# PREDICT-EPFL/polympc

Measured on AMD Instinct MI355X. Metric: box-ADMM QP subproblem solves/s (fused SQP hot path), higher is better.
Workload: dtype f64

## Files before the change

polympc_amd/csrc/pmpc_qp_reg.hpp:

```cpp
#pragma once
#include <hip/hip_runtime.h>
#include "pmpc_qp.hpp"

#ifndef PMPC_REG_RESIDUAL_BATCH
#define PMPC_REG_RESIDUAL_BATCH 14
#endif

namespace pmpc {

__device__ __forceinline__ double bcast_lane(double v, int lane) {
    const int lo = __builtin_amdgcn_readlane(__double2loint(v), lane);
    const int hi = __builtin_amdgcn_readlane(__double2hiint(v), lane);
    return __hiloint2double(hi, lo);
}
__device__ __forceinline__ void lds_order() { asm volatile("" ::: "memory"); }
__device__ __forceinline__ void sched_fence() { __builtin_amdgcn_sched_barrier(0); }

#ifndef PMPC_PIVOT_SETUP_FORM
#define PMPC_PIVOT_SETUP_FORM 0
#endif
__device__ __forceinline__ void pivot_lane_setup(double& a0, double& a1, double& a2, double& a3, double& a4, double& a5, double& a6, double& l,
                                                 double lk, int k) {
    asm("s_lshl_b64 exec, 1, %9\n\tv_mov_b64 %0, 0\n\tv_mov_b64 %1, 0\n\tv_mov_b64 %2, 0\n\tv_mov_b64 %3, 0\n\tv_mov_b64 %4, 0\n\tv_mov_b64 %5, 0\n\t"
        "v_mov_b64 %6, 0\n\tv_mov_b64 %7, %8\n\ts_mov_b64 exec, -1"
        : "+v"(a0), "+v"(a1), "+v"(a2), "+v"(a3), "+v"(a4), "+v"(a5), "+v"(a6), "+v"(l) : "v"(lk), "i"(k) : "scc");
}
__device__ __forceinline__ void pivot_lane_setup(double& a0, double& a1, double& a2, double& l, double lk, int k) {
#if PMPC_PIVOT_SETUP_FORM == 1
    asm volatile("s_lshl_b64 exec, 1, %5\n\tv_mov_b64 %0, 0\n\tv_mov_b64 %1, 0\n\tv_mov_b64 %2, 0\n\tv_mov_b64 %3, %4\n\ts_mov_b64 exec, -1"
        : "+v"(a0), "+v"(a1), "+v"(a2), "+v"(l) : "v"(lk), "i"(k) : "scc");
#elif PMPC_PIVOT_SETUP_FORM == 2
    unsigned long long saved, win;
    asm volatile("s_mov_b64 %4, exec\n\ts_lshl_b64 %5, 1, %7\n\ts_and_b64 exec, %4, %5\n\tv_mov_b64 %0, 0\n\tv_mov_b64 %1, 0\n\tv_mov_b64 %2, 0\n\tv_mov_b64 %3, %6\n\ts_mov_b64 exec, %4"
        : "+v"(a0), "+v"(a1), "+v"(a2), "+v"(l), "=&s"(saved), "=&s"(win) : "v"(lk), "i"(k) : "scc");
#elif PMPC_PIVOT_SETUP_FORM == 3
    const bool me = lane_id() == k;
    a0 = me ? 0.0 : a0; a1 = me ? 0.0 : a1; a2 = me ? 0.0 : a2; l = me ? lk : l;
#else
    asm("s_lshl_b64 exec, 1, %5\n\tv_mov_b64 %0, 0\n\tv_mov_b64 %1, 0\n\tv_mov_b64 %2, 0\n\tv_mov_b64 %3, %4\n\ts_mov_b64 exec, -1"
        : "+v"(a0), "+v"(a1), "+v"(a2), "+v"(l) : "v"(lk), "i"(k) : "scc");
#endif
}
__device__ __forceinline__ double recip_uniform(double d) {
    double y = __builtin_amdgcn_rcp(d);
    y = fma(fma(-d, y, 1.0), y, y);
    y = fma(fma(-d, y, 1.0), y, y);
    y = fma(fma(-d, y, 1.0), y, y);
    return __builtin_amdgcn_div_fixup(y, d, 1.0);
}

template <int J>
__device__ __forceinline__ double fmac_rowbcast(double acc, double x, double w) {
    asm("v_fmac_f64_dpp %0, %1, %2 row_newbcast:%3 row_mask:0xf bank_mask:0xf" : "+v"(acc) : "v"(x), "v"(w), "i"(J));
    return acc;
}
__device__ __forceinline__ void swap32(double& a, double& b) {
    const auto lo = __builtin_amdgcn_permlane32_swap(__double2loint(a), __double2loint(b), false, false);
    const auto hi = __builtin_amdgcn_permlane32_swap(__double2hiint(a), __double2hiint(b), false, false);
    a = __hiloint2double(hi[0], lo[0]); b = __hiloint2double(hi[1], lo[1]);
}
__device__ __forceinline__ void swap16(double& a, double& b) {
    const auto lo = __builtin_amdgcn_permlane16_swap(__double2loint(a), __double2loint(b), false, false);
    const auto hi = __builtin_amdgcn_permlane16_swap(__double2hiint(a), __double2hiint(b), false, false);
    a = __hiloint2double(hi[0], lo[0]); b = __hiloint2double(hi[1], lo[1]);
}

template <int N>
struct RegKkt {
    double a[((N + 15) / 16) * 16];
    using d4 = double __attribute__((ext_vector_type(4)));
    static constexpr int BK = 4;
    static constexpr int SG = 8;
    static constexpr int NB = (N + BK - 1) / BK;
    static constexpr int NT = (N + 15) / 16;
    static constexpr int NP = NT * 16;
    static constexpr int SK = 80;
    static constexpr int SX = SG + 1;
    static constexpr int XSZ = (64 * SX + 64 > BK * SK) ? 64 * SX + 64 : BK * SK;
    static constexpr int SY = 78;
    static constexpr int TRI = (BK * SK + XSZ > 16 * SY) ? BK * SK + XSZ : 16 * SY;
    static_assert(N <= 64 && SK % 32 == 16 && SK >= 64, "panel stride");
    static_assert(16 * SY <= TRI && BK % 4 == 0 && 16 % BK == 0 && BK <= SG, "conversion buffer fits the staging; block size divides a tile");

    struct NoPre { template <class TT> __device__ __forceinline__ void operator()(TT&, double*, double*, int, int, int) const {} };
    template <int NLIVE>
    __device__ __forceinline__ static double diag_abs_max(const d4 (&T)[NT][NT], int lr, int lc) {
        double dm = 0.0;
#pragma unroll
        for (int R = 0; R < (NLIVE + 15) / 16; ++R)
#pragma unroll
            for (int r = 0; r < 4; ++r) dm = fmax(dm, (lc == lr + 4 * r && 16 * R + lc < NLIVE) ? fabs(T[R][R][r]) : 0.0);
        return wave_max(dm);
    }
    template <int MM, class ALoad, class RhoOf>
    __device__ __forceinline__ static void rank_update(d4 (&T)[NT][NT], int ln, int lr, int lc, double* PA, double* PB, ALoad aload, RhoOf rho_of) {
        constexpr int NGR = (MM + 3) / 4, GB = 4;
        int z = 0;
        asm volatile("" : "+v"(z));
#pragma unroll
        for (int g0 = 0; g0 < NGR; g0 += GB) {
            double av_[GB * 4];
#pragma unroll
            for (int u = 0; u < GB * 4; ++u) { const int j = 4 * g0 + u; av_[u] = (j < MM) ? aload(j < MM ? j : 0, z) : 0.0; }
            sched_fence();
#pragma unroll
            for (int gg = 0; gg < GB; ++gg) {
                if (g0 + gg < NGR) {
#pragma unroll
                    for (int t = 0; t < 4; ++t) {
                        const int j = 4 * (g0 + gg) + t;
                        const double rj = (j < MM) ? rho_of(j < MM ? j : 0) : 0.0;
                        PB[t * SK + ln] = av_[gg * 4 + t];
                        PA[t * SK + ln] = rj * av_[gg * 4 + t];
                    }
                    lds_order();
                    double av[NT], bv[NT];
#pragma unroll
                    for (int R = 0; R < NT; ++R) { av[R] = PA[lr * SK + 16 * R + lc]; bv[R] = PB[lr * SK + 16 * R + lc]; }
                    bool nz[NT]; double probe = 0.0;
#pragma unroll
                    for (int R = 0; R < NT; ++R) { nz[R] = __builtin_amdgcn_ballot_w64(bv[R] != 0.0) != 0; probe += (av[R] - av[R]) + (bv[R] - bv[R]); }
                    const bool all = __builtin_amdgcn_ballot_w64(probe != 0.0) != 0;
#pragma unroll
                    for (int R = 0; R < NT; ++R)
#pragma unroll
                        for (int C = 0; C <= R; ++C)
                            if (all || (nz[R] && nz[C])) T[R][C] = __builtin_amdgcn_mfma_f64_16x16x4f64(av[R], bv[C], T[R][C], 0, 0, 0);
                    sched_fence();
                    lds_order();
                }
            }
        }
    }
    template <int NPIV = N, bool EST = false, class KCol, class Pre = NoPre>
    __device__ __forceinline__ bool invert(int ln_in, double* st, double diag, KCol kcol, long long* tm = nullptr, double rho_self = 0.0, Pre pre = Pre(), const double gate = PMPC_COND_GATE) {
        constexpr bool CF = NPIV < N;
        constexpr int NBP = (NPIV + BK - 1) / BK;
        long long tq0 = tm ? clock64() : 0;
        int ln = ln_in;
        asm volatile("" : "+v"(ln));
        double* PA = st;
        double* PB = st + BK * SK;
        double* X = PB;
        const int lr = ln >> 4, lc = ln & 15;
        d4 T[NT][NT];
        X[64 * SX + ln] = diag;
        sched_fence();
        int z = 0;
        asm volatile("" : "+v"(z));
#pragma unroll
        for (int j = 0; j < NP; ++j) a[j] = (j < N) ? kcol(j < N ? j : 0, z) : 0.0;
        sched_fence();
        const bool isPl = ln < NPIV;
        if constexpr (CF) {
#pragma unroll
            for (int j = 0; j < NPIV; ++j) { const double sc = -(rho_self * a[j]); a[j] = isPl ? a[j] : sc; }
        }
#pragma unroll
        for (int g = 0; g < NP / SG; ++g) {
#pragma unroll
            for (int t = 0; t < SG; ++t) {
                double v = a[g * SG + t];
                if constexpr (CF) {
                    if (g * SG + t >= NPIV && g * SG + t < N && 16 * ((g * SG + t) / 16) < NPIV) { const double sc = -(bcast_lane(rho_self, (g * SG + t < N) ? g * SG + t : 0) * v); v = isPl ? sc : v; }
                }
                X[ln * SX + t] = v;
            }
            lds_order();
            if ((lc >> 3) == (g % 2)) {
#pragma unroll
                for (int R = g / 2; R < NT; ++R)
#pragma unroll
                    for (int r = 0; r < 4; ++r) T[R][g / 2][r] = X[(16 * R + lr + 4 * r) * SX + (lc & 7)];
            }
            lds_order();
            sched_fence();
        }
#pragma unroll
        for (int R = 0; R < NT; ++R) {
            const double dR = X[64 * SX + 16 * R + lc];
#pragma unroll
            for (int r = 0; r < 4; ++r) T[R][R][r] = (lc == lr + 4 * r) ? dR : T[R][R][r];
        }
        lds_order();
        if constexpr (CF) {
            constexpr int MC = N - NPIV, KS = (MC + 3) / 4, NTP = (NPIV + 15) / 16;
#pragma unroll
            for (int s2 = 0; s2 < KS; ++s2) {
#pragma unroll
                for (int t = 0; t < 4; ++t) {
                    const int j = 4 * s2 + t;
                    const double raw = (j < MC) ? a[(NPIV + j < NP) ? NPIV + j : 0] : 0.0;
                    const double rj = (j < MC) ? bcast_lane(rho_self, (NPIV + j < N) ? NPIV + j : 0) : 0.0;
                    const double pa = rj * raw;
                    PA[t * SK + ln] = (isPl && j < MC) ? pa : 0.0;
                    PB[t * SK + ln] = (isPl && j < MC) ? raw : 0.0;
                }
                lds_order();
                double av[NTP], bv[NTP];
#pragma unroll
                for (int R = 0; R < NTP; ++R) { av[R] = PA[lr * SK + 16 * R + lc]; bv[R] = PB[lr * SK + 16 * R + lc]; }
#pragma unroll
                for (int R = 0; R < NTP; ++R)
#pragma unroll
                    for (int C = 0; C <= R; ++C) T[R][C] = __builtin_amdgcn_mfma_f64_16x16x4f64(av[R], bv[C], T[R][C], 0, 0, 0);
                sched_fence();
                lds_order();
            }
        }
        pre(T, PA, PB, ln, lr, lc);
        if constexpr (EST) { X[64 * SX + ln] = diag_abs_max<NPIV>(T, lr, lc); lds_order(); }
        if (tm) { long long t = clock64(); tm[0] += t - tq0; tq0 = t; }
#pragma unroll
        for (int b = 0; b < NBP; ++b) {
            const int kb = b * BK;
            const int w = (NPIV - kb < BK) ? NPIV - kb : BK;
            const int Cb = kb / 16, hb = (kb % 16) / BK;
            constexpr int RPB = BK / 4;
            if ((lc / BK) == hb) {
#pragma unroll
                for (int R = Cb; R < NT; ++R)
#pragma unroll
                    for (int r = 0; r < 4; ++r) X[(16 * R + lr + 4 * r) * SX + (lc % BK)] = T[R][Cb][r];
            }
#pragma unroll
            for (int C = 0; C < Cb; ++C)
#pragma unroll
                for (int rr = 0; rr < RPB; ++rr) X[(16 * C + lc) * SX + lr + 4 * rr] = T[Cb][C][RPB * hb + rr];
            lds_order();
            double p[BK];
#pragma unroll
            for (int t = 0; t < BK; ++t) p[t] = X[ln * SX + t];
            lds_order();
            const bool inb = (ln / BK) == b && (!CF || ln < NPIV);
            if (tm) { long long t = clock64(); tm[1] += t - tq0; tq0 = t; }
#pragma unroll
            for (int t = 0; t < BK; ++t) PB[t * SK + ln] = (inb || kb + t >= NPIV) ? 0.0 : p[t];
#pragma unroll
            for (int t = 0; t < BK; ++t) {
                const int k = kb + t;
                if (k < NPIV) {
                    const double dk = bcast_lane(p[t], k);
                    const double r = recip_uniform(dk);
                    double rk[BK];
#pragma unroll
                    for (int u = 0; u < BK; ++u) rk[u] = (u != t && u < w) ? bcast_lane(p[u], k) : 0.0;
                    double l = p[t] * r;
                    if (w == BK) {
                        if constexpr (BK == 8) pivot_lane_setup(p[(t + 1) & 7], p[(t + 2) & 7], p[(t + 3) & 7], p[(t + 4) & 7], p[(t + 5) & 7], p[(t + 6) & 7], p[(t + 7) & 7], l, -r, k);
                        else pivot_lane_setup(p[(t + 1) & 3], p[(t + 2) & 3], p[(t + 3) & 3], l, -r, k);
                    } else {
#pragma unroll
                        for (int u = 0; u < BK; ++u) if (u != t && u < w) p[u] = (ln == k) ? 0.0 : p[u];
                        l = (ln == k) ? -r : l;
                    }
#pragma unroll
                    for (int u = 0; u < BK; ++u)
                        if (u != t && u < w) p[u] = fma(-l, rk[u], p[u]);
                    p[t] = l;
                    sched_fence();
                }
            }
            if (tm) { long long t = clock64(); tm[2] += t - tq0; tq0 = t; }
#pragma unroll
            for (int t = 0; t < BK; ++t) PA[t * SK + ln] = (inb || kb + t >= NPIV) ? 0.0 : -p[t];
            lds_order();
#pragma unroll
            for (int s2 = 0; s2 < BK / 4; ++s2) {
                double av[NT], bv[NT];
#pragma unroll
                for (int R = 0; R < NT; ++R) {
                    av[R] = PA[(4 * s2 + lr) * SK + 16 * R + lc];
                    bv[R] = PB[(4 * s2 + lr) * SK + 16 * R + lc];
                }
#pragma unroll
                for (int R = 0; R < NT; ++R)
#pragma unroll
                    for (int C = 0; C <= R; ++C) T[R][C] = __builtin_amdgcn_mfma_f64_16x16x4f64(av[R], bv[C], T[R][C], 0, 0, 0);
                sched_fence();
            }
            lds_order();
            if (tm) { long long t = clock64(); tm[3] += t - tq0; tq0 = t; }
#pragma unroll
            for (int t = 0; t < BK; ++t) X[ln * SX + t] = p[t];
            lds_order();
            if ((lc / BK) == hb && (lc % BK) < w) {
#pragma unroll
                for (int R = Cb; R < NT; ++R)
#pragma unroll
                    for (int r = 0; r < 4; ++r) T[R][Cb][r] = X[(16 * R + lr + 4 * r) * SX + (lc % BK)];
            }
#pragma unroll
            for (int C = 0; C <= Cb; ++C)
#pragma unroll
                for (int rr = 0; rr < RPB; ++rr) {
                    const double xv_ = X[(16 * C + lc) * SX + lr + 4 * rr];
                    T[Cb][C][RPB * hb + rr] = (w == BK || lr + 4 * rr < w) ? xv_ : T[Cb][C][RPB * hb + rr];
                }
            lds_order();
            sched_fence();
        }
        if (tm) { long long t = clock64(); tm[1] += t - tq0; tq0 = t; }
        if constexpr (EST) {
            const double smax = X[64 * SX + ln];
            const double wmax = diag_abs_max<NPIV>(T, lr, lc);
            if (__builtin_amdgcn_readfirstlane((int)(smax * wmax > gate))) return true;
        }
        double* Y = st;
#pragma unroll
        for (int q = 0; q < NT; ++q) {
#pragma unroll
            for (int C = 0; C < NT; ++C) {
                if (C <= q) {
#pragma unroll
                    for (int r = 0; r < 4; ++r) Y[(lr + 4 * r) * SY + 16 * C + lc] = T[q][C][r];
                } else {
#pragma unroll
                    for (int r = 0; r < 4; ++r) Y[lc * SY + 16 * C + lr + 4 * r] = T[C][q][r];
                }
            }
            lds_order();
            const int yo = lc * SY + 16 * (lr < NT ? lr : 0);
#pragma unroll
            for (int j = 0; j < 16; ++j) {
                const double y = Y[yo + j];
                a[16 * q + j] = (16 * (NT - 1) + j < N && NT == 4) ? y : ((16 * lr + j < N) ? y : 0.0);
            }
            lds_order();
            sched_fence();
        }
        if (tm) { long long t = clock64(); tm[4] += t - tq0; tq0 = t; }
        return false;
    }

    __device__ __forceinline__ double apply(double c) const {
        double acc[4] = {0.0, 0.0, 0.0, 0.0};
        asm volatile("s_nop 1" : "+v"(c));
        unroll_j<0>(acc, c);
        asm volatile("s_nop 1" : "+v"(acc[0]), "+v"(acc[1]), "+v"(acc[2]), "+v"(acc[3]));
        swap32(acc[0], acc[2]);
        swap32(acc[1], acc[3]);
        double s0 = acc[0] + acc[2], s1 = acc[1] + acc[3];
        swap16(s0, s1);
        return -(s0 + s1);
    }
    template <int J>
    __device__ __forceinline__ void unroll_j(double (&acc)[4], double c) const {
        if constexpr (J < 16) {
#pragma unroll
            for (int q = 0; q < NT; ++q) acc[q] = fmac_rowbcast<J>(acc[q], c, a[16 * q + J]);
            unroll_j<J + 1>(acc, c);
        }
    }
};

template <int NN, int MM, bool STACKED = false, bool SYMLOWER = false, bool GATE = false>
__device__ __forceinline__ void boxadmm_solve_reg(const double* __restrict__ H, const double* h, const double* __restrict__ A,
                                                  const double* Alb, const double* Aub, const double* xlb, const double* xub,
                                                  const double* x0, const double* y0, const pmpc_qp_settings& s, pmpc_qp_info& info,
                                                  double* out_x, double* out_y, double* tr, long long* dbg = nullptr, long long* tm = nullptr) {
    constexpr int N = NN + MM;
    static_assert(N <= WAVE, "register-resident path needs n+m <= 64");
    const long long tp0 = dbg ? clock64() : 0;
    const int ln = lane_id();
    const bool isP = ln < NN;
    const bool isC = (ln >= NN) && (ln < N);
    const int r = isC ? ln - NN : 0;

    const int lp = isP ? ln : 0;
    const double hv = isP ? h[lp] : 0.0;
    const double lo = isP ? xlb[lp] : (isC ? Alb[r] : 0.0);
    const double hi = isP ? xub[lp] : (isC ? Aub[r] : 0.0);
    const int type = classify_bounds(lo, hi);

    const double* rowp = isP ? (H + ln) : (A + r);
    const int rstride = isP ? NN : (isC ? MM : 0);
    const double* colA = A + (size_t)lp * MM;
    const unsigned roff = (ln < N) ? ln : 0, coff = lp * N + NN;
    auto lane_near = [](int zo) -> unsigned { unsigned l; asm("v_mbcnt_lo_u32_b32 %0, -1, 0\n\tv_mbcnt_hi_u32_b32 %0, -1, %0" : "=&v"(l) : "v"(zo)); return l; };
    auto Krow = [&](int j, int zo) -> double {
        if constexpr (STACKED) { const unsigned l = lane_near(zo); unsigned b = (l < (unsigned)N ? l : 0u) + (unsigned)zo; asm("" : "+v"(b)); return H[b + (unsigned)(j * N)]; }
        else return rowp[(size_t)j * (size_t)(unsigned)(rstride + zo)];
    };
    auto KrowLower = [&](int j, int zo) -> double {
        if constexpr (STACKED) {
            const unsigned l = lane_near(zo);
            const unsigned lc = (l < (unsigned)N ? l : 0u);
            unsigned b = ((lc < (unsigned)j) ? ((unsigned)j + lc * (unsigned)N) : (lc + (unsigned)(j * N))) + (unsigned)zo;
            asm("" : "+v"(b));
            return H[b];
        } else {
            const bool up = isP && ln < j;
            const double* src = up ? H + ((size_t)lp * NN + (size_t)(unsigned)(j + zo)) : rowp + (size_t)j * (size_t)(unsigned)(rstride + zo);
            return *src;
        }
    };
    auto Acol = [&](int k, int zo) -> double {
        if constexpr (STACKED) { const unsigned l = lane_near(zo); unsigned b = (l < (unsigned)NN ? l : 0u) * N + NN + (unsigned)zo; asm("" : "+v"(b)); return H[b + (unsigned)k]; }
        else return colA[k + zo];
    };
    constexpr int LDH = STACKED ? N : NN;

    double xv = 0.0, yv = 0.0, qv = 0.0;
    {
        const double x0v = x0 ? x0[lp] : 0.0, ybv = y0 ? y0[MM + lp] : 0.0, yav = y0 ? y0[r] : 0.0;
        xv = isP ? x0v : 0.0; qv = xv; yv = isP ? ybv : (isC ? yav : 0.0);
    }
    if (x0) {
        double acc = 0.0;
#pragma unroll
        for (int j = 0; j < NN; ++j) acc += Krow(j, 0) * bcast_lane(xv, j);
        xv = isC ? acc : xv;
    }

    double rho = s.rho;
    int rho_updates = 1;
    double rhov = rho_of(type, rho);
    double rhoinv = 1.0 / rhov;
    double kdiag;
    {
        double kd = H[(size_t)lp * LDH + lp]; kd += s.sigma; kd += rhov;
        kdiag = isP ? kd : rhov;
    }

    RegKkt<N> K;
    int status = PMPC_QP_UNSOLVED;
    constexpr int GAVE_UP = 100;
    const double alpha = s.alpha;
    double max_Ax_z_norm = 0.0, max_Hx_ATy_h_norm = 0.0, res_prim = 1.0, res_dual = 1.0, rho_estimate = 0.0;
    int iter = 1;
    int until_check = s.check_termination, until_adapt = s.adaptive_rho_interval;
    bool running = true;
    if (dbg) dbg[17] += clock64() - tp0;
    while (running) {
        {
            const long long f0 = dbg ? clock64() : 0;
            const bool tripped = K.template invert<NN, GATE>(ln, tr, kdiag, [&](int j, int z) -> double {
                if (j < NN) { if constexpr (SYMLOWER) return KrowLower(j < NN ? j : 0, z); else return Krow(j < NN ? j : 0, z); }
                const double v = Acol(j >= NN ? j - NN : 0, z);
                if constexpr (STACKED) return lane_near(z) < (unsigned)NN ? v : 0.0;
                return isP ? v : 0.0;
            }, tm, rhov);
            if constexpr (GATE) { if (tripped) { status = GAVE_UP; running = false; if (dbg) dbg[0] += clock64() - f0; break; } }
            if (dbg) dbg[0] += clock64() - f0;
        }
        bool refactor = false;
        for (; iter <= s.max_iter; ++iter) {
            const long long ti0 = dbg ? clock64() : 0;
            const double zprev = xv;
            const double rhsP = ((s.sigma * xv - hv) + rhov * qv) - yv;
            const double rhsC = xv - rhoinv * yv;
            const double rhs = isP ? rhsP : (isC ? rhsC : 0.0);
            const double sol = K.apply(rhs);
            const double zt = zprev + rhoinv * (sol - yv);
            double zz = alpha * zt;
            zz += (1 - alpha) * zprev + rhoinv * yv;
            zz = fmin(fmax(zz, lo), hi);
            const double yC = yv + rhov * ((alpha * zt + (1 - alpha) * zprev) - zz);
            double xx = alpha * sol;
            xx += (1 - alpha) * xx;
            double qq = xx + rhoinv * yv;
            qq = fmin(fmax(qq, lo), hi);
            const double yP = yv + rhov * (xx - qq);
            xv = isP ? xx : (isC ? zz : xv);
            qv = isP ? qq : qv;
            yv = isP ? yP : (isC ? yC : yv);
            if (dbg) dbg[9] += clock64() - ti0;
            bool check = false, adapt = false;
            if (s.check_termination != 0 && --until_check == 0) { check = true; until_check = s.check_termination; }
            if (s.adaptive_rho && --until_adapt == 0) { adapt = true; until_adapt = s.adaptive_rho_interval; }
            if (check || adapt) {
                const long long r0 = dbg ? clock64() : 0;
                constexpr int RC = PMPC_REG_RESIDUAL_BATCH;
                int zr = 0;
                asm volatile("" : "+v"(zr));
                double acc = 0.0;
                double aty = 0.0;
#pragma unroll
                for (int e0 = 0; e0 < N; e0 += RC) {
                    double mv[RC];
#pragma unroll
                    for (int e = 0; e < RC; ++e) {
                        const int ee = e0 + e;
                        mv[e] = (ee < NN) ? Krow(ee < NN ? ee : 0, zr) : ((ee < N) ? Acol((ee >= NN && ee < N) ? ee - NN : 0, zr) : 0.0);
                    }
#pragma unroll
                    for (int e = 0; e < RC; ++e) {
                        const int ee = e0 + e;
                        if (ee < NN) acc += mv[e] * bcast_lane(xv, ee);
                        else if (ee < N) aty += mv[e] * bcast_lane(yv, ee);
                    }
                    sched_fence();
                }
                const double ax = fabs(xv);
                max_Ax_z_norm = wave_max(isC ? fmax(fabs(acc), ax) : (isP ? ax : 0.0));
                max_Hx_ATy_h_norm = wave_max(isP ? fmax(fmax(fabs(acc), fabs(aty)), fmax(fabs(hv), fabs(yv))) : 0.0);
                const double rp = wave_max(isC ? fabs(acc - xv) : 0.0), rq = wave_max(isP ? fabs(xv - qv) : 0.0);
                res_prim = rp + rq;
                res_dual = wave_max(isP ? fabs(((acc + hv) + aty) + yv) : 0.0);
                if (dbg) dbg[1] += clock64() - r0;
            }
            if (check) {
                const double ep = s.eps_abs + s.eps_rel * max_Ax_z_norm, ed = s.eps_abs + s.eps_rel * max_Hx_ATy_h_norm;
                if (__builtin_amdgcn_readfirstlane((int)(res_prim <= ep && res_dual <= ed))) { status = PMPC_QP_SOLVED; running = false; break; }
            }
            if (adapt) {
                const double rpn = res_prim / (max_Ax_z_norm + DIV_BY_ZERO_REGUL);
                const double rdn = res_dual / (max_Hx_ATy_h_norm + DIV_BY_ZERO_REGUL);
                double new_rho = rho * ::sqrt(rpn / (rdn + DIV_BY_ZERO_REGUL));
                new_rho = fmax(RHO_MIN, fmin(new_rho, RHO_MAX));
                rho_estimate = new_rho;
                if (__builtin_amdgcn_readfirstlane((int)(new_rho < rho / s.adaptive_rho_tolerance || new_rho > rho * s.adaptive_rho_tolerance))) {
                    const double prev = rhov;
                    rho = new_rho;
                    rhov = rho_of(type, rho);
                    rhoinv = 1.0 / rhov;
                    ++rho_updates;
                    kdiag = isP ? (kdiag + (rhov - prev)) : rhov;
                    refactor = true;
                    ++iter;
                    break;
                }
            }
        }
        if (!refactor) running = false;
    }
    const bool gave_up = GATE && status == GAVE_UP;
    if (gave_up) status = PMPC_QP_UNSOLVED;
    else if (iter > s.max_iter) status = PMPC_QP_MAX_ITER_EXCEEDED;
    if (isP) { out_x[ln] = xv; out_y[MM + ln] = yv; }
    if (isC) out_y[r] = yv;
    const bool bad = __builtin_amdgcn_ballot_w64(((xv - xv) + (yv - yv)) != 0.0) != 0;
    info.status = status; info.iter = iter; info.rho_updates = rho_updates; info.flags = (bad ? PMPC_FLAG_NONFINITE : 0) | (gave_up ? PMPC_FLAG_ILLCOND : 0);
    info.rho_estimate = rho_estimate; info.res_prim = res_prim; info.res_dual = res_dual;
}

}
```

Measured before the change: 28.20 million.

## Load KKT tiles directly from global memory into MFMA fragment layout

For the stacked, non-gated path, the KKT matrix tiles are now read straight from the workspace into the per-lane MFMA accumulator layout. This bypasses the per-lane row loads followed by the LDS transpose staging through X. The constraint-first rho scaling and the off-diagonal panel for the Schur update are also loaded directly, and rho is broadcast through LDS. The change removes LDS round trips and barriers in the factorization setup. In exchange it issues more scattered global loads and adds complex index and masking logic.

```diff
diff --git a/polympc_amd/csrc/pmpc_qp_reg.hpp b/polympc_amd/csrc/pmpc_qp_reg.hpp
--- a/polympc_amd/csrc/pmpc_qp_reg.hpp
+++ b/polympc_amd/csrc/pmpc_qp_reg.hpp
@@ -64,6 +64,20 @@
     const auto hi = __builtin_amdgcn_permlane16_swap(__double2hiint(a), __double2hiint(b), false, false);
     a = __hiloint2double(hi[0], lo[0]); b = __hiloint2double(hi[1], lo[1]);
 }
+
+__device__ __forceinline__ unsigned lane_id_near(int zo) {
+    unsigned l;
+    asm("v_mbcnt_lo_u32_b32 %0, -1, 0\n\tv_mbcnt_hi_u32_b32 %0, -1, %0" : "=&v"(l) : "v"(zo));
+    return l;
+}
+
+#ifndef PMPC_DIRECT_STAGING
+#define PMPC_DIRECT_STAGING 3
+#endif
+template <class KCol>
+struct StackedTileSource { const double* ws; KCol kcol; };
+template <class T> struct is_stacked_tile_source { static constexpr bool value = false; };
+template <class KCol> struct is_stacked_tile_source<StackedTileSource<KCol>> { static constexpr bool value = true; };
 
 template <int N>
 struct RegKkt {
@@ -145,17 +159,65 @@
         const int lr = ln >> 4, lc = ln & 15;
         d4 T[NT][NT];
         X[64 * SX + ln] = diag;
+        constexpr bool DIRECT = is_stacked_tile_source<KCol>::value;
+        constexpr int DS = DIRECT ? PMPC_DIRECT_STAGING : 0;
+        static_assert(!DIRECT || (CF && !EST && BK * SK + XSZ + 64 <= TRI), "direct tile staging: constraint-first mode without the conditioning gate");
+        constexpr int MCD = N - NPIV, KSD = (MCD + 3) / 4, NTPD = (NPIV + 15) / 16;
+        double* RH = st + BK * SK + XSZ;
+        if constexpr (DS >= 2) RH[ln] = rho_self;
+        auto rowsP = [](int R, int r) constexpr { return 16 * R + 4 * r + 3 < NPIV; };
+        auto rowsC = [](int R, int r) constexpr { return 16 * R + 4 * r >= NPIV; };
+        auto colsP = [](int C) constexpr { return 16 * C + 15 < NPIV; };
+        auto direct = [&](int R, int C, int r) constexpr { return DS >= 2 || (DS == 1 && rowsP(R, r) && colsP(C)); };
         sched_fence();
         int z = 0;
         asm volatile("" : "+v"(z));
-#pragma unroll
-        for (int j = 0; j < NP; ++j) a[j] = (j < N) ? kcol(j < N ? j : 0, z) : 0.0;
+        auto&& rowload = [&]() -> auto& { if constexpr (DIRECT) return kcol.kcol; else return kcol; }();
+        if constexpr (DS < 2) {
+#pragma unroll
+            for (int j = 0; j < NP; ++j) a[j] = (j < N) ? rowload(j < N ? j : 0, z) : 0.0;
+        } else if constexpr (DS == 2) {
+#pragma unroll
+            for (int j = NPIV; j < N; ++j) a[j] = rowload(j, z);
+        }
+        [[maybe_unused]] double ov[DS == 3 ? KSD * NTPD : 1];
+        if constexpr (DS >= 1) {
+            const unsigned l = lane_id_near(z), dlr = l >> 4, dlc = l & 15;
+            unsigned bP = dlr * N + dlc + (unsigned)z, bC = dlc * N + dlr + (unsigned)z;
+            asm("" : "+v"(bP));
+            asm("" : "+v"(bC));
+#pragma unroll
+            for (int R = 0; R < NT; ++R)
+#pragma unroll
+                for (int C = 0; C <= R; ++C)
+#pragma unroll
+                    for (int r = 0; r < 4; ++r) {
+                        if (!direct(R, C, r)) continue;
+                        const int i0 = 16 * R + 4 * r, j0 = 16 * C;
+                        const unsigned oP = (j0 + 15 < N) ? bP + (unsigned)(i0 * N + j0) : (j0 + dlc < (unsigned)N ? bP + (unsigned)(i0 * N + j0) : 0u);
+                        const unsigned iC = (i0 + 3 < N) ? bC + (unsigned)i0 : (i0 >= N ? bC - dlr : (i0 + dlr < (unsigned)N ? bC + (unsigned)i0 : bC - dlr));
+                        const unsigned oC = colsP(C) ? iC + (unsigned)(j0 * N) : (j0 + dlc < (unsigned)NPIV ? iC + (unsigned)(j0 * N) : 0u);
+                        const unsigned o = rowsP(R, r) ? oP : (rowsC(R, r) ? oC : (i0 + dlr < (unsigned)NPIV ? oP : oC));
+                        T[R][C][r] = kcol.ws[o];
+                    }
+            if constexpr (DS == 3) {
+#pragma unroll
+                for (int s2 = 0; s2 < KSD; ++s2)
+#pragma unroll
+                    for (int R = 0; R < NTPD; ++R) {
+                        const bool in = (4 * s2 + 3 < MCD || 4 * s2 + dlr < (unsigned)MCD) && (16 * R + 15 < NPIV || 16 * R + dlc < (unsigned)NPIV);
+                        const unsigned o = in ? bC + (unsigned)(16 * R * N + NPIV + 4 * s2) : 0u;
+                        ov[s2 * NTPD + R] = kcol.ws[o];
+                    }
+            }
+        }
         sched_fence();
         const bool isPl = ln < NPIV;
-        if constexpr (CF) {
+        if constexpr (CF && DS < 2) {
 #pragma unroll
             for (int j = 0; j < NPIV; ++j) { const double sc = -(rho_self * a[j]); a[j] = isPl ? a[j] : sc; }
         }
+        if constexpr (DS < 2) {
 #pragma unroll
         for (int g = 0; g < NP / SG; ++g) {
 #pragma unroll
@@ -171,10 +233,32 @@
 #pragma unroll
                 for (int R = g / 2; R < NT; ++R)
 #pragma unroll
-                    for (int r = 0; r < 4; ++r) T[R][g / 2][r] = X[(16 * R + lr + 4 * r) * SX + (lc & 7)];
+                    for (int r = 0; r < 4; ++r) if (!direct(R, g / 2, r)) T[R][g / 2][r] = X[(16 * R + lr + 4 * r) * SX + (lc & 7)];
             }
             lds_order();
             sched_fence();
+        }
+        } else {
+            lds_order();
+#pragma unroll
+            for (int R = 0; R < NT; ++R) {
+                const double rhoc = (16 * R < NPIV && 16 * R + 15 >= NPIV) ? RH[16 * R + lc] : 0.0;
+#pragma unroll
+                for (int r = 0; r < 4; ++r) {
+                    const int i0 = 16 * R + 4 * r;
+                    const bool rowP = rowsP(R, r) || (!rowsC(R, r) && i0 + lr < NPIV);
+                    const double rhor = rowsP(R, r) ? 0.0 : RH[i0 + lr];
+#pragma unroll
+                    for (int C = 0; C <= R; ++C) {
+                        const int j0 = 16 * C;
+                        const double v = T[R][C][r];
+                        const double vP = colsP(C) ? v : (j0 + lc < NPIV ? v : ((j0 + 15 < N || j0 + lc < N) ? -(rhoc * v) : 0.0));
+                        const double sc = -(rhor * v);
+                        const double vC = colsP(C) ? sc : (j0 + lc < NPIV ? sc : 0.0);
+                        T[R][C][r] = rowsP(R, r) ? vP : (rowsC(R, r) ? vC : (rowP ? vP : vC));
+                    }
+                }
+            }
         }
 #pragma unroll
         for (int R = 0; R < NT; ++R) {
@@ -185,6 +269,25 @@
         lds_order();
         if constexpr (CF) {
             constexpr int MC = N - NPIV, KS = (MC + 3) / 4, NTP = (NPIV + 15) / 16;
+            if constexpr (DS == 3) {
+#pragma unroll
+                for (int s2 = 0; s2 < KS; ++s2) {
+                    const bool jin = 4 * s2 + 3 < MC || 4 * s2 + lr < MC;
+                    const double rj = RH[NPIV + (jin ? 4 * s2 + lr : 0)];
+                    double av[NTP], bv[NTP];
+#pragma unroll
+                    for (int R = 0; R < NTP; ++R) {
+                        const bool in = jin && (16 * R + 15 < NPIV || 16 * R + lc < NPIV);
+                        const double raw = ov[s2 * NTP + R], pa = rj * raw;
+                        av[R] = in ? pa : 0.0; bv[R] = in ? raw : 0.0;
+                    }
+#pragma unroll
+                    for (int R = 0; R < NTP; ++R)
+#pragma unroll
+                        for (int C = 0; C <= R; ++C) T[R][C] = __builtin_amdgcn_mfma_f64_16x16x4f64(av[R], bv[C], T[R][C], 0, 0, 0);
+                    sched_fence();
+                }
+            } else {
 #pragma unroll
             for (int s2 = 0; s2 < KS; ++s2) {
 #pragma unroll
@@ -206,6 +309,7 @@
                     for (int C = 0; C <= R; ++C) T[R][C] = __builtin_amdgcn_mfma_f64_16x16x4f64(av[R], bv[C], T[R][C], 0, 0, 0);
                 sched_fence();
                 lds_order();
+            }
             }
         }
         pre(T, PA, PB, ln, lr, lc);
@@ -435,12 +539,15 @@
     while (running) {
         {
             const long long f0 = dbg ? clock64() : 0;
-            const bool tripped = K.template invert<NN, GATE>(ln, tr, kdiag, [&](int j, int z) -> double {
+            auto kcol = [&](int j, int z) -> double {
                 if (j < NN) { if constexpr (SYMLOWER) return KrowLower(j < NN ? j : 0, z); else return Krow(j < NN ? j : 0, z); }
                 const double v = Acol(j >= NN ? j - NN : 0, z);
                 if constexpr (STACKED) return lane_near(z) < (unsigned)NN ? v : 0.0;
                 return isP ? v : 0.0;
-            }, tm, rhov);
+            };
+            bool tripped;
+            if constexpr (STACKED && !SYMLOWER && !GATE && PMPC_DIRECT_STAGING != 0) tripped = K.template invert<NN, GATE>(ln, tr, kdiag, StackedTileSource<decltype(kcol)>{H, kcol}, tm, rhov);
+            else tripped = K.template invert<NN, GATE>(ln, tr, kdiag, kcol, tm, rhov);
             if constexpr (GATE) { if (tripped) { status = GAVE_UP; running = false; if (dbg) dbg[0] += clock64() - f0; break; } }
             if (dbg) dbg[0] += clock64() - f0;
         }
```

Measured after the change: 29.18 million, median of 6. 3.5% higher.
